# PhilippKath/concentus

Measured on AMD Instinct MI355X. Metric: 48kHz stereo 20ms CELT frames encoded/sec, higher is better.
Workload: dtype int16/int32 fixed-point

## Files before the change

concentus_amd/csrc/celt_enc.h:

```cpp
#pragma once
#include "celt_enc_back.h"

namespace ca {

struct FrameResult { int bytes; u32 final_range; };

template <class L>
CA_DEV void load_state(FrameCtx &fc, L &F, const opusgpu_celt_state *st, int C)
{
    fc.C = C;
    if (st) {
        for (int k = 0; k < 4; k++) fc.hp_mem[k] = st->hp_mem[k];
        fc.rng = st->rng;
        fc.spread_decision = st->spread_decision;
        fc.delayedIntra = st->delayedIntra;
        fc.tonal_average = st->tonal_average;
        fc.lastCodedBands = st->lastCodedBands;
        fc.hf_average = st->hf_average;
        fc.tapset_decision = st->tapset_decision;
        fc.prefilter_period = st->prefilter_period;
        fc.prefilter_gain = st->prefilter_gain;
        fc.prefilter_tapset = st->prefilter_tapset;
        fc.consec_transient = st->consec_transient;
        fc.preemph_memE[0] = st->preemph_memE[0];
// ... 363 lines not shown
    if (!L::IN_IS_GLOBAL)
        for (int c = 0; c < C; c++)
            for (int i = lane(); i < N + OVL; i += LANES) tsig(F, c)[i] = in_ws[c * (N + OVL) + i];
    wave_sync();
  }
  if constexpr (PHASE != 1) {
    int isTransient = 0, shortBlocks = 0, tf_chan = 0, transient_got_disabled = 0;
    i32 tf_estimate = 0;
    if (cfg.complexity >= 1) {
        TransientOut to;
        if constexpr (PHASE == 2) {
            i32 um[2] = {uni(mid->trans_unmask[0]), uni(mid->trans_unmask[1])};
            to = transient_combine(um, C);
        } else {
            to = transient_analysis_wave(F, fc);
        }
        isTransient = to.is_transient;
        tf_estimate = to.tf_estimate;
        tf_chan = to.tf_chan;
    }
    if (ec_tell(enc) + 3 <= total_bits) {
        if (isTransient) shortBlocks = M;
    } else {
        isTransient = 0;
        transient_got_disabled = 1;
    }

    CA_TRACE("transient done isT=%d tf_est=%d", isTransient, tf_estimate); CA_TRACE("");
    CA_STAMP(4);
    const int secondMdct = shortBlocks && cfg.complexity >= 8;
    i32 temporal_vbr = 0;
    for (int mdct_pass = secondMdct ? 0 : 1;;) {
        CA_STAMP(5);
        if constexpr (L::XF_CHANNELS == 1) {
            for (int c = 0; c < C; c++) {
                compute_mdct_channel(F, c, mdct_pass == 0 ? 0 : shortBlocks);
                band_energies_channel(F, c, mdct_pass == 0 ? F.bandLogE2 : F.bandLogE);
                if (mdct_pass != 0) normalise_bands_channel(F, c);
            }
        } else {
            compute_mdcts_wave(F, fc, mdct_pass == 0 ? 0 : shortBlocks);
            CA_STAMP(30);
            band_energies_wave(F, fc, mdct_pass == 0 ? F.bandLogE2 : F.bandLogE);
        }
        CA_STAMP(31);
        if (mdct_pass == 0) {
            for (int k = lane(); k < C * NB; k += LANES) F.bandLogE2[k] = (i16)(F.bandLogE2[k] + (shl16(LM, 10) >> 1));
            wave_sync();
            mdct_pass = 1;
            continue;
        }
        if (mdct_pass == 2) {
            for (int k = lane(); k < C * NB; k += LANES) F.bandLogE2[k] = (i16)(F.bandLogE2[k] + (shl16(LM, 10) >> 1));
            wave_sync();
            tf_estimate = 3277;
            break;
        }
        if constexpr (L::XF_CHANNELS != 1) CA_TAP("freq", F.xf, sizeof(F.xf));
        CA_TAP("bandE", F.bandE, sizeof(F.bandE)); CA_TAP("bandLogE", F.bandLogE, sizeof(F.bandLogE));
        {
            i32 follow = -10240;
            i32 frame_avg = 0;
            i32 offset = shortBlocks ? (shl16(LM, 10) >> 1) : 0;
            for (int i = 0; i < end; i++) {
                follow = (i16)imax(follow - 1024, F.bandLogE[i] - offset);
                if (C == 2) follow = (i16)imax(follow, F.bandLogE[i + NB] - offset);
                frame_avg += follow;
            }
            frame_avg /= end;
            temporal_vbr = (i16)sub16(frame_avg, fc.spec_avg);
            temporal_vbr = imin(3072, imax(-1536, temporal_vbr));
            fc.spec_avg = (i16)(fc.spec_avg + mul16_16_q15(655, temporal_vbr));
        }
        if (!secondMdct) {
            for (int k = lane(); k < C * NB; k += LANES) F.bandLogE2[k] = F.bandLogE[k];
            wave_sync();
        }
        if (!(ec_tell(enc) + 3 <= total_bits && !isTransient && cfg.complexity >= 5)) break;
        i16 *spread_old = F.follower;
        if (lane() == 0) {
            if (C == 1) {
                spread_old[0] = F.oldBandE[0];
                for (int i = 1; i < end; i++) spread_old[i] = (i16)imax(spread_old[i - 1] - 1024, F.oldBandE[i]);
            } else {
                spread_old[0] = (i16)imax(F.oldBandE[0], F.oldBandE[NB]);
                for (int i = 1; i < end; i++)
                    spread_old[i] = (i16)imax(spread_old[i - 1] - 1024, imax(F.oldBandE[i], F.oldBandE[i + NB]));
            }
            for (int i = end - 2; i >= 0; i--) spread_old[i] = (i16)imax(spread_old[i], spread_old[i + 1] - 1024);
        }
        wave_sync();
        i32 mean_diff = 0;
        for (int c = 0; c < C; c++)
            for (int i = 2; i < end - 1; i++) {
                i32 x1 = imax(0, F.bandLogE[i + c * NB]), x2 = imax(0, spread_old[i]);
                mean_diff = add32(mean_diff, imax(0, sub16(x1, x2)));
            }
        mean_diff = mean_diff / (C * (end - 1 - 2));
        wave_sync();
        if (!(mean_diff > 1024)) break;
        isTransient = 1;
        shortBlocks = M;
        mdct_pass = 2;
    }
    if (ec_tell(enc) + 3 <= total_bits) ec_enc_bit_logp(enc, isTransient, 3);

    CA_STAMP(5);
    if constexpr (L::XF_CHANNELS != 1) normalise_bands_wave(F, fc);

    if constexpr (!L::IN_IS_GLOBAL) CA_TAP("X", F.in, 2 * FRAME * 2);
    CA_STAMP(6);
    {
        const i16 *X = frame_X(F);
        if (X != mid->X)
            for (int k = lane(); k < 2 * FRAME; k += LANES) mid->X[k] = X[k];
        MidScalars m;
        m.max_data_bytes = max_data_bytes; m.nbCompressedBytes = nbCompressedBytes; m.nbAvailableBytes = nbAvailableBytes;
        m.effectiveBytes = effectiveBytes; m.vbr_rate = vbr_rate; m.equiv_rate = equiv_rate; m.total_bits = total_bits;
        m.silence = silence; m.pitch_index = pitch_index; m.pf_on = pf_on; m.prefilter_tapset = prefilter_tapset; m.gain1 = gain1;
        m.isTransient = isTransient; m.shortBlocks = shortBlocks; m.tf_chan = tf_chan;
        m.transient_got_disabled = transient_got_disabled; m.tf_estimate = tf_estimate; m.temporal_vbr = temporal_vbr;
        mid_store(F, mid, enc, fc, m);
    }
  }
}

template <class L>
CA_DEVFN void celt_encode_front(L &F, const opusgpu_celt_config &cfg, const opusgpu_celt_state *st_in,
                                opusgpu_celt_state *st_out, const i16 *pcm, FrameMid *mid, StageClock *stage_clock = nullptr)
{
    celt_encode_front_phase<0>(F, cfg, st_in, st_out, pcm, mid, stage_clock, nullptr);
}

template <class L>
CA_DEVFN FrameResult celt_encode_back(L &F, const opusgpu_celt_config &cfg, const FrameMid *mid, opusgpu_celt_state *st_out,
                                      u8 *out, StageClock *stage_clock = nullptr)
{
    (void)stage_clock;
    if (lane() == 0) F.diag = (void *)stage_clock;
    const int C = 2, LM = LM3, end = NB;
    const int celt_vbr = cfg.vbr, constrained_vbr = cfg.constrained_vbr;
// ... 321 lines not shown
```

concentus_amd/csrc/celt_enc_front.h:

```cpp
#pragma once
#include <stddef.h>
#include "celt_math.h"
#include "celt_state.h"
#include "device_tables.h"
#include "mdct_dev.h"
#include "rangecoder.h"

namespace ca {

#if defined(CA_HOST_EMU)
#define CA_DEVFN static inline
#else
#define CA_DEVFN __device__ __forceinline__
#endif

enum { NB = 21, OVL = 120, FRAME = 960, MAXP = 1024, MINP = 15, LM3 = 3, M8 = 8 };
enum { SPREAD_NONE = 0, SPREAD_LIGHT = 1, SPREAD_NORMAL = 2, SPREAD_AGGRESSIVE = 3 };

template <class P, class V> CA_DEV void st0(P p, V v) { if (lane() == 0) *p = v; }

struct __attribute__((aligned(16))) FrontLds {
    enum { IN_IS_GLOBAL = 0, XF_CHANNELS = 2 };
    i32 in[2][FRAME + OVL];
    i32 xf[2][FRAME];
    union {
        i16 raw_pcm[2 * FRAME];
        struct { i16 buf[992]; i16 xlp4[240]; i16 ylp4[484]; i32 xcorr[520]; } pitch;
        i16 trans[2][FRAME + OVL];
        int2 f2[480];
    } s;
    u8 packet[64];
    i32 bandE[2 * NB];
    i16 bandLogE[2 * NB], bandLogE2[2 * NB];
    i16 oldBandE[2 * NB], oldLogE[2 * NB], oldLogE2[2 * NB];
    i16 follower[2 * NB];
    i16 normg[2 * NB];
    i8 normshift[2 * NB];
    i32 scal[16];
    void *diag;
};

#if defined(CA_LANE_FRAME)
enum { LS_SLOTS = 264, LS_PULSES = 240 };
struct FrameMid;
struct BackLds {
    x16_t *x16;
    u8 *packet;
    CA_AS_LDS i16 *col;
    FrameMid *mid;
    void *diag;
    u32 tf_bits;
    int tf_sel;
    u32 ps0[4], ps1[4], ps2[4];
};
#else
struct __attribute__((aligned(16))) BackLds {
    i16 x16[2 * FRAME];
    union {
        struct { i16 tmp[176]; i16 tmp1[176]; } tf;
        struct { i16 y[176]; i32 iy[176]; i16 xabs[176]; } pvq;
    } s;
    u8 packet[1280];
    i32 bandE[2 * NB];
    i16 bandLogE[2 * NB], bandLogE2[2 * NB], error[2 * NB];
    i16 oldBandE[2 * NB], oldLogE[2 * NB], oldLogE2[2 * NB];
    i16 oldE_intra[2 * NB], error_intra[2 * NB];
    i16 follower[2 * NB], noise_floor[NB];
    u8 coarse_save[256];
    i32 offsets[NB], cap[NB], pulses[NB], fine_quant[NB], fine_priority[NB], tf_res[NB];
    i32 bits1[NB], bits2[NB], thresh[NB], trim_offset[NB];
    i32 metric[NB], path0[NB], path1[NB];
    i32 scal[16];
    void *diag;
    i32 pstack[4][8];
};
#endif

struct __attribute__((aligned(16))) Front1Lds {
    enum { IN_IS_GLOBAL = 1, XF_CHANNELS = 2 };
    i32 *in_g;
    i32 xf[2][FRAME];
    union {
        struct { i16 buf[992]; i16 xlp4[240]; i16 ylp4[484]; i32 xcorr[520]; } pitch;
    } s;
    u8 packet[64];
    i32 bandE[2 * NB];
    i16 bandLogE[2 * NB], bandLogE2[2 * NB];
    i16 oldBandE[2 * NB], oldLogE[2 * NB], oldLogE2[2 * NB];
    i32 scal[16];
    void *diag;
};

struct __attribute__((aligned(16))) Front2Lds {
    enum { IN_IS_GLOBAL = 1, XF_CHANNELS = 1 };
    i32 *in_g;
    i16 *x_g;
    i32 xf[1][FRAME];
    union {
        int2 f2[480];
    } s;
    u8 packet[64];
    i32 bandE[2 * NB];
    i16 bandLogE[2 * NB], bandLogE2[2 * NB];
    i16 oldBandE[2 * NB], oldLogE[2 * NB], oldLogE2[2 * NB];
    i16 follower[2 * NB];
    i16 normg[2 * NB];
    i8 normshift[2 * NB];
    i32 scal[16];
    void *diag;
};

CA_DEV i32 *tsig(FrontLds &F, int c) { return F.in[c]; }
CA_DEV i32 *tsig(Front1Lds &F, int c) { return F.in_g + c * (FRAME + OVL); }
CA_DEV i32 *tsig(Front2Lds &F, int c) { return F.in_g + c * (FRAME + OVL); }

CA_DEV i16 *frame_X(FrontLds &F) { return reinterpret_cast<i16 *>(&F.in[0][0]); }
CA_DEV i16 *frame_X(Front2Lds &F) { return F.x_g; }
CA_DEV i16 *frame_pcmf(Front1Lds &F) { return reinterpret_cast<i16 *>(&F.xf[0][0]); }
CA_DEV x16_t *frame_X(BackLds &F) { return F.x16; }
CA_DEV i16 *frame_pcmf(FrontLds &F) { return reinterpret_cast<i16 *>(&F.xf[0][0]); }

struct FrameCtx {
    int C;
    i32 hp_mem[4];
    u32 rng;
    int spread_decision, tonal_average, lastCodedBands, hf_average, tapset_decision;
    i32 delayedIntra;
    int prefilter_period, prefilter_gain, prefilter_tapset, consec_transient;
    i32 preemph_memE[2];
    i32 vbr_reservoir, vbr_drift, vbr_offset, vbr_count, overlap_max;
    int stereo_saving, intensity, spec_avg;
    int stereo_narrow;
    const i32 *hist;
// ... 670 lines not shown
            mean = add32(mean, x2);
            tmp[i] = (i16)(mem0 + pshr32(x2 - mem0, 4));
            mem0 = tmp[i];
        }
        mem0 = 0;
        i32 maxE = 0;
        for (int i = len2 - 1; i >= 0; i--) {
            tmp[i] = (i16)(mem0 + pshr32(tmp[i] - mem0, 3));
            mem0 = tmp[i];
            maxE = imax(maxE, mem0);
        }
        mean = mul16_16(celt_sqrt(mean), celt_sqrt(mul16_16(maxE, len2 >> 1)));
        i32 norm = shl32(len2, 6 + 14) / add32(1, mean >> 1);
        F.scal[4 + c] = norm;
    }
    wave_sync();
    i32 um[2] = {0, 0};
    for (int c = 0; c < C; c++) {
        const i16 *tmp = F.s.trans[c];
        i32 norm = F.scal[4 + c];
        i32 p = 0;
        for (int k = lane(); 12 + 4 * k < len2 - 5; k += LANES) {
            int i = 12 + 4 * k;
            i32 id = imax(0, imin(127, mul16_32_q15((i16)(tmp[i] + 1), norm)));
            p += CLT_inv_table[id];
        }
        i32 unmask = wave_add(p);
        um[c] = 64 * unmask * 4 / (6 * (len2 - 17));
    }
    wave_sync();
    return transient_combine(um, C);
}

template <class L> CA_DEV i32 *xf_row(L &F, int c) { return F.xf[L::XF_CHANNELS == 1 ? 0 : c]; }

template <class L>
CA_DEVFN void compute_mdct_channel(L &F, int c, int shortBlocks)
{
    if (shortBlocks) {
        const MdctTab T = mdct_global_tab<3>();
        mdct_forward_wave<3, 8>(tsig(F, c), F.s.f2, xf_row(F, c), 1, T, lane());
    } else {
        const MdctTab T = mdct_global_tab<0>();
        mdct_forward_wave<0, 1>(tsig(F, c), F.s.f2, xf_row(F, c), 1, T, lane());
    }
}

template <class L>
CA_DEVFN void compute_mdcts_wave(L &F, const FrameCtx &fc, int shortBlocks)
{
    for (int c = 0; c < fc.C; c++) compute_mdct_channel(F, c, shortBlocks);
}

template <class L>
CA_DEVFN void band_energies_channel(L &F, int c, i16 *bandLogE)
{
    const i32 *X = xf_row(F, c);
    i32 *red = reinterpret_cast<i32 *>(F.s.f2);
    constexpr int NCH = 100;
    for (int ch = lane(); ch < NCH; ch += LANES) {
        i32 mx = 0, mn = 0;
#pragma unroll
        for (int u = 0; u < 8; u++) { const i32 v = X[8 * ch + u]; mx = imax(mx, v); mn = imin(mn, v); }
        red[ch] = mx;
        red[NCH + ch] = mn;
    }
    wave_sync();
// ... 34 lines not shown

template <class L>
CA_DEVFN void band_energies_wave(L &F, const FrameCtx &fc, i16 *bandLogE)
{
    for (int c = 0; c < fc.C; c++) band_energies_channel(F, c, bandLogE);
}

template <class L>
CA_DEVFN void normalise_bands_channel(L &F, int c)
{
    i16 *X = frame_X(F);
    const i32 *xf = xf_row(F, c);
    for (int k = c * NB + lane(); k < (c + 1) * NB; k += LANES) {
        i32 bE = F.bandE[k];
        int shift = celt_zlog2(bE) - 13;
        i32 E = (i16)vshr32(bE, shift);
        F.normg[k] = (i16)celt_rcp(shl32(E, 3));
        F.normshift[k] = (i8)shift;
    }
    wave_sync();
    for (int j = lane(); j < (CLT_eband5ms[NB] << LM3); j += LANES) {
        int b = CLT_bin2band[j >> 3] + c * NB;
        X[c * FRAME + j] = (i16)mul16_16_q15(vshr32(xf[j], F.normshift[b] - 1), F.normg[b]);
    }
    wave_sync();
}

template <class L>
CA_DEVFN void normalise_bands_wave(L &F, const FrameCtx &fc)
{
    for (int c = 0; c < fc.C; c++) normalise_bands_channel(F, c);
}

}
```

concentus_amd/csrc/celt_enc_kernel.hip:

```cpp
#include "celt_enc.h"
#include "opusgpu_internal.h"

namespace ca {

__global__ __launch_bounds__(64, 3) void celt_front1_kernel(opusgpu_celt_config cfg, opusgpu_celt_state *states,
                                                            FrameMid *__restrict__ mid, i32 *__restrict__ in_ws, int nframes)
{
    __shared__ Front1Lds F;
    for (int n = blockIdx.x; n < nframes; n += gridDim.x) {
        opusgpu_celt_state *st = states ? states + n : nullptr;
        i32 *in = in_ws + (size_t)n * 2 * (FRAME + OVL);
        if (lane() == 0) F.in_g = in;
        wave_sync();
        celt_encode_front_phase<1>(F, cfg, st, st, nullptr, mid + n, nullptr, in);
        wave_sync();
    }
}

__global__ __launch_bounds__(64, 4) void celt_front2_kernel(opusgpu_celt_config cfg, FrameMid *__restrict__ mid,
                                                            i32 *__restrict__ in_ws, int nframes)
{
    __shared__ Front2Lds F;
    for (int n = blockIdx.x; n < nframes; n += gridDim.x) {
        i32 *in = in_ws + (size_t)n * 2 * (FRAME + OVL);
        if (lane() == 0) { F.in_g = in; F.x_g = mid[n].X; }
        wave_sync();
        celt_encode_front_phase<2>(F, cfg, nullptr, nullptr, nullptr, mid + n, nullptr, in);
        wave_sync();
    }
}

__global__ void celt_state_init_kernel(opusgpu_celt_state *states, int n)
{
    int i = blockIdx.x;
    if (i >= n) return;
    u32 *w = reinterpret_cast<u32 *>(&states[i]);
    for (int k = threadIdx.x; k < (int)(sizeof(opusgpu_celt_state) / 4); k += blockDim.x) w[k] = 0;
    __syncthreads();
    if (threadIdx.x == 0) {
        states[i].spread_decision = SPREAD_NORMAL;
        states[i].delayedIntra = 1;
        states[i].tonal_average = 256;
    }
    for (int k = threadIdx.x; k < 2 * NB; k += blockDim.x) {
        states[i].oldLogE[k] = -28672;
        states[i].oldLogE2[k] = -28672;
    }
}

}

// ... 106 lines not shown
```

concentus_amd/csrc/mdct_dev.h:

```cpp
#pragma once
#include "fixmath.h"
#include "device_tables.h"

namespace ca {

struct MdctTab {
    const u32 *tw;
    const u32 *trig;
    const i16 *bitrev;
    const i16 *window;
    const i16 *bitrev_sw;
};

template <int SHIFT>
CA_DEV MdctTab mdct_global_tab()
{
    MdctTab t;
    t.tw = CLT_fft_tw_packed;
    t.trig = SHIFT == 0 ? CLT_mdct_trig_packed0 : SHIFT == 1 ? CLT_mdct_trig_packed1
           : SHIFT == 2 ? CLT_mdct_trig_packed2 : CLT_mdct_trig_packed3;
    t.bitrev = SHIFT == 0 ? CLT_fft_bitrev480 : SHIFT == 1 ? CLT_fft_bitrev240
             : SHIFT == 2 ? CLT_fft_bitrev120 : CLT_fft_bitrev60;
    t.window = CLT_window120;
    t.bitrev_sw = CLT_fft_bitrev480_sw;
// ... 17 lines not shown
    for (int i = tid; i < 120; i += nthreads) L.window[i] = g.window[i];
    MdctTab t;
    t.tw = L.tw; t.trig = L.trig; t.bitrev = L.bitrev; t.window = L.window;
    t.bitrev_sw = g.bitrev_sw;
    return t;
}

struct cpx { i32 r, i; };
CA_DEV cpx ld(const int2 *p) { int2 v = *p; return cpx{v.x, v.y}; }
CA_DEV void st(int2 *p, cpx v) { *p = make_int2(v.r, v.i); }
CA_DEV i32 lo16(u32 p) { return (i32)(i16)(p & 0xffff); }
CA_DEV i32 hi16(u32 p) { return (i32)p >> 16; }
#define CA_SMUL(x, t) mul16_32_q15((t), (x))

CA_DEV cpx c_mul(cpx a, u32 tw)
{
    i32 tr = lo16(tw), ti = hi16(tw);
    cpx m;
    m.r = sub32(CA_SMUL(a.r, tr), CA_SMUL(a.i, ti));
    m.i = add32(CA_SMUL(a.r, ti), CA_SMUL(a.i, tr));
    return m;
}
CA_DEV cpx c_add(cpx a, cpx b) { return cpx{add32(a.r, b.r), add32(a.i, b.i)}; }
CA_DEV cpx c_sub(cpx a, cpx b) { return cpx{sub32(a.r, b.r), sub32(a.i, b.i)}; }

#if defined(CA_HOST_EMU)
#define CA_FFT_ROLLED
CA_DEV int fft_lane(int lane) { return lane; }
#else
#define CA_FFT_ROLLED _Pragma("clang loop unroll(disable)")
CA_DEV int fft_lane(int lane) { asm volatile("" : "+v"(lane)); return lane; }
#endif

template <int SHIFT>
CA_DEV int fsw(int e)
{
    if constexpr (SHIFT == 0) {
        constexpr unsigned long long LUT = CLT_FSW_LUT;
        const int s = (int)(LUT >> ((e >> 3) & 60)) & 30;
        return e ^ s ^ ((e >> 2) & 4);
    } else {
        return e;
    }
}

template <int SW, int P, int M>
CA_DEV void fft_members(int e, int (&a)[P])
{
    if constexpr (SW != 0) {
#pragma unroll
        for (int c = 0; c < P; c++) a[c] = e + c * M;
    } else if constexpr (M == 8) {
        const int A = e ^ ((int)(CLT_FSW_LUT >> ((e >> 3) & 60)) & 30);
#pragma unroll
        for (int c = 0; c < P; c++) a[c] = A ^ ((8 * c) ^ (4 * (c >> 1)));
    } else {
        static_assert(M % 32 == 0, "members whole blocks apart");
        const unsigned long long W = CLT_FSW_LUT >> ((e >> 3) & 60);
        const int E = e ^ ((e >> 2) & 4);
#pragma unroll
        for (int c = 0; c < P; c++) a[c] = (E + c * M) ^ ((int)(W >> (4 * ((c * M) >> 5))) & 30);
    }
}

struct cpx2 { cpx a, b; };
CA_DEV cpx2 ld2(const int2 *p)
{
    const int4 v = *reinterpret_cast<const int4 *>(p);
    return cpx2{cpx{v.x, v.y}, cpx{v.z, v.w}};
}
CA_DEV void st2(int2 *p, cpx a, cpx b)
{
    int4 v;
    v.x = a.r; v.y = a.i; v.z = b.r; v.w = b.i;
    *reinterpret_cast<int4 *>(p) = v;
}

template <int NFFT, int B>
CA_DEV void fft_radix4_first(int2 *x, int lane)
{
    constexpr int CNT = B * NFFT / 4;
    for (int idx = lane; idx < CNT; idx += LANES) {
        int2 *f = x + 4 * idx;
        cpx x0 = ld(f), x1 = ld(f + 1), x2 = ld(f + 2), x3 = ld(f + 3);
        cpx s0 = c_sub(x0, x2);
        x0 = c_add(x0, x2);
        cpx s1 = c_add(x1, x3);
        x2 = c_sub(x0, s1);
        x0 = c_add(x0, s1);
        s1 = c_sub(x1, x3);
        st(f, x0);
        st(f + 2, x2);
        st(f + 1, cpx{add32(s0.r, s1.i), sub32(s0.i, s1.r)});
        st(f + 3, cpx{sub32(s0.r, s1.i), add32(s0.i, s1.r)});
    }
}

template <int NFFT, int B>
CA_DEV void fft_radix2_m4(int2 *x, int lane)
{
    constexpr int CNT = B * NFFT / 2;
    constexpr i32 TW = 23170;
    for (int idx = lane; idx < CNT; idx += LANES) {
        int g = idx >> 2, k = idx & 3;
        int2 *f = x + 8 * g + k;
        cpx a = ld(f), b = ld(f + 4), t;
        if (k == 0) {
            t = b;
        } else if (k == 1) {
            t.r = CA_SMUL(add32(b.r, b.i), TW);
            t.i = CA_SMUL(sub32(b.i, b.r), TW);
        } else if (k == 2) {
            t.r = b.i;
            t.i = neg32(b.r);
        } else {
            t.r = CA_SMUL(sub32(b.i, b.r), TW);
            t.i = CA_SMUL(sub32(neg32(b.i), b.r), TW);
        }
        st(f + 4, c_sub(a, t));
        st(f, c_add(a, t));
    }
}

template <int SHIFT>
CA_DEV void fft_first8(int2 *x, int lane)
{
    constexpr int NFFT = 480 >> SHIFT;
    constexpr i32 TW = 23170;
    lane = fft_lane(lane);
    for (int g = lane; g < NFFT / 8; g += LANES) {
        cpx v[8];
        const int A = fsw<SHIFT>(8 * g);
#pragma unroll
        for (int q = 0; q < 4; q++) {
            const cpx2 t = ld2(x + (A ^ (2 * q)));
            v[2 * q] = t.a;
            v[2 * q + 1] = t.b;
        }
#pragma unroll
        for (int h = 0; h < 2; h++) {
            cpx x0 = v[4 * h], x1 = v[4 * h + 1], x2 = v[4 * h + 2], x3 = v[4 * h + 3];
            cpx s0 = c_sub(x0, x2);
            x0 = c_add(x0, x2);
            cpx s1 = c_add(x1, x3);
            x2 = c_sub(x0, s1);
            x0 = c_add(x0, s1);
            s1 = c_sub(x1, x3);
            v[4 * h] = x0;
            v[4 * h + 2] = x2;
            v[4 * h + 1] = cpx{add32(s0.r, s1.i), sub32(s0.i, s1.r)};
            v[4 * h + 3] = cpx{sub32(s0.r, s1.i), add32(s0.i, s1.r)};
        }
        {
            cpx t, b;
            b = v[4]; t = b;
            v[4] = c_sub(v[0], t); v[0] = c_add(v[0], t);
            b = v[5]; t.r = CA_SMUL(add32(b.r, b.i), TW); t.i = CA_SMUL(sub32(b.i, b.r), TW);
            v[5] = c_sub(v[1], t); v[1] = c_add(v[1], t);
            b = v[6]; t.r = b.i; t.i = neg32(b.r);
            v[6] = c_sub(v[2], t); v[2] = c_add(v[2], t);
            b = v[7]; t.r = CA_SMUL(sub32(b.i, b.r), TW); t.i = CA_SMUL(sub32(neg32(b.i), b.r), TW);
            v[7] = c_sub(v[3], t); v[3] = c_add(v[3], t);
        }
#pragma unroll
        for (int q = 0; q < 4; q++) st2(x + (A ^ (2 * q)), v[2 * q], v[2 * q + 1]);
    }
}

template <int NFFT, int B, int M>
CA_DEV void fft_radix4(int2 *x, const u32 *tw, int lane)
{
    constexpr int G = NFFT / (4 * M);
    constexpr int TWS = G * (480 / NFFT);
    constexpr int CNT = B * NFFT / 4;
    constexpr int SW = (NFFT == 480 && B == 1) ? 0 : 1;
    lane = fft_lane(lane);
    CA_FFT_ROLLED
    for (int idx = lane; idx < CNT; idx += LANES) {
        int blk = idx / (G * M), r = idx % (G * M);
        int g = r / M, j = r % M;
        const int e = blk * NFFT + g * 4 * M + j;
        int m[4];
        fft_members<SW, 4, M>(e, m);
        int2 *f0p = x + m[0], *f1p = x + m[1], *f2p = x + m[2], *f3p = x + m[3];
        cpx f0 = ld(f0p);
        cpx a = c_mul(ld(f1p), tw[j * TWS]);
        cpx b = c_mul(ld(f2p), tw[2 * j * TWS]);
        cpx c = c_mul(ld(f3p), tw[3 * j * TWS]);
        cpx d5 = c_sub(f0, b);
        f0 = c_add(f0, b);
        cpx s3 = c_add(a, c);
        cpx s4 = c_sub(a, c);
        st(f2p, c_sub(f0, s3));
        st(f0p, c_add(f0, s3));
        st(f1p, cpx{add32(d5.r, s4.i), sub32(d5.i, s4.r)});
        st(f3p, cpx{sub32(d5.r, s4.i), add32(d5.i, s4.r)});
    }
}

template <int NFFT, int B, int M>
CA_DEV void fft_radix3(int2 *x, const u32 *tw, int lane)
{
    constexpr int G = NFFT / (3 * M);
    constexpr int TWS = G * (480 / NFFT);
    constexpr int CNT = B * NFFT / 3;
    constexpr int SW = (NFFT == 480 && B == 1) ? 0 : 1;
    constexpr i32 EPI3 = -28378;
    lane = fft_lane(lane);
    CA_FFT_ROLLED
    for (int idx = lane; idx < CNT; idx += LANES) {
        int blk = idx / (G * M), r = idx % (G * M);
        int g = r / M, j = r % M;
        const int e = blk * NFFT + g * 3 * M + j;
        int m[3];
        fft_members<SW, 3, M>(e, m);
        int2 *f0p = x + m[0], *f1p = x + m[1], *f2p = x + m[2];
        cpx f0 = ld(f0p);
        cpx a = c_mul(ld(f1p), tw[j * TWS]);
        cpx b = c_mul(ld(f2p), tw[2 * j * TWS]);
        cpx s3 = c_add(a, b);
        cpx s0 = c_sub(a, b);
        cpx f1{sub32(f0.r, s3.r >> 1), sub32(f0.i, s3.i >> 1)};
        s0.r = CA_SMUL(s0.r, EPI3);
        s0.i = CA_SMUL(s0.i, EPI3);
        st(f0p, c_add(f0, s3));
        st(f2p, cpx{add32(f1.r, s0.i), sub32(f1.i, s0.r)});
        st(f1p, cpx{sub32(f1.r, s0.i), add32(f1.i, s0.r)});
    }
}

template <int NFFT, int B, int M>
CA_DEV void fft_radix5(int2 *x, const u32 *tw, int lane)
{
    constexpr int G = NFFT / (5 * M);
    constexpr int TWS = G * (480 / NFFT);
    constexpr int CNT = B * NFFT / 5;
    constexpr int SW = (NFFT == 480 && B == 1) ? 0 : 1;
    constexpr i32 YAR = 10126, YAI = -31164, YBR = -26510, YBI = -19261;
    lane = fft_lane(lane);
    CA_FFT_ROLLED
    for (int idx = lane; idx < CNT; idx += LANES) {
        int blk = idx / (G * M), r = idx % (G * M);
        int g = r / M, u = r % M;
        const int e = blk * NFFT + g * 5 * M + u;
        int m[5];
        fft_members<SW, 5, M>(e, m);
        int2 *f0p = x + m[0], *f1p = x + m[1], *f2p = x + m[2], *f3p = x + m[3], *f4p = x + m[4];
        cpx s0 = ld(f0p);
        cpx s1 = c_mul(ld(f1p), tw[u * TWS]);
        cpx s2 = c_mul(ld(f2p), tw[2 * u * TWS]);
        cpx s3 = c_mul(ld(f3p), tw[3 * u * TWS]);
        cpx s4 = c_mul(ld(f4p), tw[4 * u * TWS]);
        cpx s7 = c_add(s1, s4), s10 = c_sub(s1, s4);
        cpx s8 = c_add(s2, s3), s9 = c_sub(s2, s3);
        st(f0p, cpx{add32(s0.r, add32(s7.r, s8.r)), add32(s0.i, add32(s7.i, s8.i))});
        cpx s5, s6, s11, s12;
        s5.r = add32(add32(s0.r, CA_SMUL(s7.r, YAR)), CA_SMUL(s8.r, YBR));
        s5.i = add32(add32(s0.i, CA_SMUL(s7.i, YAR)), CA_SMUL(s8.i, YBR));
        s6.r = add32(CA_SMUL(s10.i, YAI), CA_SMUL(s9.i, YBI));
        s6.i = sub32(neg32(CA_SMUL(s10.r, YAI)), CA_SMUL(s9.r, YBI));
        st(f1p, c_sub(s5, s6));
        st(f4p, c_add(s5, s6));
        s11.r = add32(add32(s0.r, CA_SMUL(s7.r, YBR)), CA_SMUL(s8.r, YAR));
        s11.i = add32(add32(s0.i, CA_SMUL(s7.i, YBR)), CA_SMUL(s8.i, YAR));
        s12.r = add32(neg32(CA_SMUL(s10.i, YBI)), CA_SMUL(s9.i, YAI));
        s12.i = sub32(CA_SMUL(s10.r, YBI), CA_SMUL(s9.r, YAI));
        st(f2p, c_add(s11, s12));
        st(f3p, c_sub(s11, s12));
    }
}

template <int SHIFT, int B> CA_DEV int fft_at(int e) { return fsw<(SHIFT == 0 && B == 1) ? 0 : 1>(e); }
template <int SHIFT, int B> CA_DEV void fft_put(int2 *x, int e, cpx v) { st(x + fft_at<SHIFT, B>(e), v); }
template <int SHIFT, int B> CA_DEV cpx fft_get(const int2 *x, int e) { return ld(x + fft_at<SHIFT, B>(e)); }

template <int SHIFT, int B>
CA_DEV void fft_wave(int2 *x, const u32 *tw, int lane)
{
    constexpr int NFFT = 480 >> SHIFT;
    if constexpr (SHIFT == 0 && B == 1) {
        fft_first8<0>(x, lane);                 wave_sync();
        fft_radix4<NFFT, B, 8>(x, tw, lane);    wave_sync();
        fft_radix3<NFFT, B, 32>(x, tw, lane);   wave_sync();
        fft_radix5<NFFT, B, 96>(x, tw, lane);   wave_sync();
        return;
    }
    fft_radix4_first<NFFT, B>(x, lane);
    wave_sync();
    if constexpr (SHIFT == 0) {
        fft_radix2_m4<NFFT, B>(x, lane);        wave_sync();
        fft_radix4<NFFT, B, 8>(x, tw, lane);    wave_sync();
        fft_radix3<NFFT, B, 32>(x, tw, lane);   wave_sync();
        fft_radix5<NFFT, B, 96>(x, tw, lane);   wave_sync();
    } else if constexpr (SHIFT == 1) {
        fft_radix4<NFFT, B, 4>(x, tw, lane);    wave_sync();
        fft_radix3<NFFT, B, 16>(x, tw, lane);   wave_sync();
        fft_radix5<NFFT, B, 48>(x, tw, lane);   wave_sync();
    } else if constexpr (SHIFT == 2) {
        fft_radix2_m4<NFFT, B>(x, lane);        wave_sync();
        fft_radix3<NFFT, B, 8>(x, tw, lane);    wave_sync();
        fft_radix5<NFFT, B, 24>(x, tw, lane);   wave_sync();
    } else {
        fft_radix3<NFFT, B, 4>(x, tw, lane);    wave_sync();
        fft_radix5<NFFT, B, 12>(x, tw, lane);   wave_sync();
    }
}

template <int SHIFT>
CA_DEV cpx mdct_fwd_pre(const i32 *in, int i, const MdctTab &T)
{
    constexpr int N2 = 960 >> SHIFT, N4 = N2 / 2;
    constexpr int OV = 120, OV2 = 60, Q = 30;
    constexpr int SCALE_SHIFT = (8 - SHIFT) - 1;
    const int a = OV2 + 2 * i, b = N2 - 1 + OV2 - 2 * i;
    i32 re, im;
    if (i < Q) {
        i32 w1 = T.window[OV2 + 2 * i], w2 = T.window[OV2 - 1 - 2 * i];
        re = add32(mul16_32_q15(w2, in[a + N2]), mul16_32_q15(w1, in[b]));
        im = sub32(mul16_32_q15(w1, in[a]), mul16_32_q15(w2, in[b - N2]));
    } else if (i < N4 - Q) {
        re = in[b];
        im = in[a];
    } else {
        int k = i - (N4 - Q);
        i32 w1 = T.window[2 * k], w2 = T.window[OV - 1 - 2 * k];
        re = add32(neg32(mul16_32_q15(w1, in[a - N2])), mul16_32_q15(w2, in[b]));
        im = add32(mul16_32_q15(w2, in[a]), mul16_32_q15(w1, in[b + N2]));
    }
    u32 t = T.trig[i];
    i32 t0 = lo16(t), t1 = hi16(t);
    i32 yr = sub32(CA_SMUL(re, t0), CA_SMUL(im, t1));
    i32 yi = add32(CA_SMUL(im, t0), CA_SMUL(re, t1));
    return cpx{pshr32(mul16_32_q16(17476, yr), SCALE_SHIFT), pshr32(mul16_32_q16(17476, yi), SCALE_SHIFT)};
}

enum { FFT_PAIRS = 240, FFT_PAIR_STEP = LANES >= 60 ? 60 : LANES };
CA_DEV int fft_pair_input(int n) { return n < 120 ? n : n + 120; }
// ... 1 lines not shown
template <int SHIFT, int B>
CA_DEV void mdct_forward_wave(const i32 *sin, int2 *f2, i32 *dst, int dstride, const MdctTab &T, int lane)
{
    const u32 *trig = T.trig;
    const i16 *bitrev = T.bitrev;
    constexpr int N2 = 960 >> SHIFT, N4 = N2 / 2, NFFT = N4;
    if constexpr (SHIFT == 0 && B == 1) {
        static_assert(FFT_PAIRS % FFT_PAIR_STEP == 0, "whole trips");
        if (lane < FFT_PAIR_STEP) {
            CA_FFT_ROLLED
            for (int n0 = 0; n0 < FFT_PAIRS; n0 += FFT_PAIR_STEP) {
                const int i = fft_pair_input(n0 + lane);
                const cpx a = mdct_fwd_pre<SHIFT>(sin, i, T), b = mdct_fwd_pre<SHIFT>(sin, i + 120, T);
                st2(f2 + T.bitrev_sw[i], a, b);
            }
        }
    } else {
        for (int idx = lane; idx < B * N4; idx += LANES) {
            int blk = idx / N4, i = idx % N4;
            fft_put<SHIFT, B>(f2, blk * NFFT + bitrev[i], mdct_fwd_pre<SHIFT>(sin + blk * N2, i, T));
        }
    }
    wave_sync();
    fft_wave<SHIFT, B>(f2, T.tw, lane);
    for (int idx = lane; idx < B * N4; idx += LANES) {
        int blk = idx / N4, i = idx % N4;
        cpx f = fft_get<SHIFT, B>(f2, blk * NFFT + i);
        u32 t = trig[i];
        i32 t0 = lo16(t), t1 = hi16(t);
        dst[((2 * i) * B + blk) * dstride] = sub32(CA_SMUL(f.i, t1), CA_SMUL(f.r, t0));
        dst[((N2 - 1 - 2 * i) * B + blk) * dstride] = add32(CA_SMUL(f.r, t1), CA_SMUL(f.i, t0));
    }
    wave_sync();
}

template <int SHIFT, int B>
CA_DEV void mdct_backward_wave(const i32 *src, int sstride, int2 *f2, i32 *out, const MdctTab &T, int lane)
{
    const u32 *trig = T.trig;
    const i16 *bitrev = T.bitrev;
    constexpr int N2 = 960 >> SHIFT, N4 = N2 / 2, NFFT = N4;
    constexpr int OV = 120, OV2 = 60;
    auto pre = [&](int blk, int i) {
        i32 x1 = src[((2 * i) * B + blk) * sstride];
        i32 x2 = src[((N2 - 1 - 2 * i) * B + blk) * sstride];
        u32 t = trig[i];
        i32 t0 = lo16(t), t1 = hi16(t);
        i32 yr = add32(CA_SMUL(x2, t0), CA_SMUL(x1, t1));
        i32 yi = sub32(CA_SMUL(x1, t0), CA_SMUL(x2, t1));
        return cpx{yi, yr};
    };
    if constexpr (SHIFT == 0 && B == 1) {
        if (lane < FFT_PAIR_STEP) {
            CA_FFT_ROLLED
            for (int n0 = 0; n0 < FFT_PAIRS; n0 += FFT_PAIR_STEP) {
                const int i = fft_pair_input(n0 + lane);
                st2(f2 + T.bitrev_sw[i], pre(0, i), pre(0, i + 120));
            }
        }
    } else {
        for (int idx = lane; idx < B * N4; idx += LANES) {
            int blk = idx / N4, i = idx % N4;
            fft_put<SHIFT, B>(f2, blk * NFFT + bitrev[i], pre(blk, i));
        }
    }
    wave_sync();
// ... 25 lines not shown
```

Before: 9.644 million.

## Process both channels jointly in front2 MDCT, band energy and normalisation

Replaces the per-channel MDCT/band-energy/normalise loop in the single-xf front2 layout with joint two-channel versions. The FFT stages take a channel-count parameter so each stage handles both channels in one wave pass, halving the number of barrier-separated stages. The MDCT output is rotated in place into the FFT buffer, which is unioned with xf. Band energies use a two-level reduction over 8-bin chunks instead of per-band serial loops. This adds LDS use (a reduction buffer and shift array, guarded by a static_assert for 16 waves per CU) and more register pressure from the staged post-rotation.

```diff
diff --git a/concentus_amd/csrc/celt_enc.h b/concentus_amd/csrc/celt_enc.h
--- a/concentus_amd/csrc/celt_enc.h
+++ b/concentus_amd/csrc/celt_enc.h
@@ -419,12 +419,12 @@
     i32 temporal_vbr = 0;
     for (int mdct_pass = secondMdct ? 0 : 1;;) {
         CA_STAMP(5);
-        if constexpr (L::XF_CHANNELS == 1) {
-            for (int c = 0; c < C; c++) {
-                compute_mdct_channel(F, c, mdct_pass == 0 ? 0 : shortBlocks);
-                band_energies_channel(F, c, mdct_pass == 0 ? F.bandLogE2 : F.bandLogE);
-                if (mdct_pass != 0) normalise_bands_channel(F, c);
-            }
+        if (mdct_pass == 2) CA_COUNT("front_mdct_redo", 1);
+        else if (mdct_pass == 1 && shortBlocks) CA_COUNT("front_mdct_short", 1);
+        if constexpr (L::JOINT_CHANNELS) {
+            compute_mdcts_joint(F, mdct_pass == 0 ? 0 : shortBlocks);
+            band_energies_joint(F, mdct_pass == 0 ? F.bandLogE2 : F.bandLogE);
+            if (mdct_pass != 0) normalise_bands_joint(F);
         } else {
             compute_mdcts_wave(F, fc, mdct_pass == 0 ? 0 : shortBlocks);
             CA_STAMP(30);
@@ -443,7 +443,7 @@
             tf_estimate = 3277;
             break;
         }
-        if constexpr (L::XF_CHANNELS != 1) CA_TAP("freq", F.xf, sizeof(F.xf));
+        if constexpr (!L::JOINT_CHANNELS) CA_TAP("freq", F.xf, sizeof(F.xf));
         CA_TAP("bandE", F.bandE, sizeof(F.bandE)); CA_TAP("bandLogE", F.bandLogE, sizeof(F.bandLogE));
         {
             i32 follow = -10240;
@@ -493,7 +493,7 @@
     if (ec_tell(enc) + 3 <= total_bits) ec_enc_bit_logp(enc, isTransient, 3);
 
     CA_STAMP(5);
-    if constexpr (L::XF_CHANNELS != 1) normalise_bands_wave(F, fc);
+    if constexpr (!L::JOINT_CHANNELS) normalise_bands_wave(F, fc);
 
     if constexpr (!L::IN_IS_GLOBAL) CA_TAP("X", F.in, 2 * FRAME * 2);
     CA_STAMP(6);
diff --git a/concentus_amd/csrc/celt_enc_front.h b/concentus_amd/csrc/celt_enc_front.h
--- a/concentus_amd/csrc/celt_enc_front.h
+++ b/concentus_amd/csrc/celt_enc_front.h
@@ -20,7 +20,7 @@
 template <class P, class V> CA_DEV void st0(P p, V v) { if (lane() == 0) *p = v; }
 
 struct __attribute__((aligned(16))) FrontLds {
-    enum { IN_IS_GLOBAL = 0, XF_CHANNELS = 2 };
+    enum { IN_IS_GLOBAL = 0, JOINT_CHANNELS = 0 };
     i32 in[2][FRAME + OVL];
     i32 xf[2][FRAME];
     union {
@@ -77,7 +77,7 @@
 #endif
 
 struct __attribute__((aligned(16))) Front1Lds {
-    enum { IN_IS_GLOBAL = 1, XF_CHANNELS = 2 };
+    enum { IN_IS_GLOBAL = 1, JOINT_CHANNELS = 0 };
     i32 *in_g;
     i32 xf[2][FRAME];
     union {
@@ -92,13 +92,15 @@
 };
 
 struct __attribute__((aligned(16))) Front2Lds {
-    enum { IN_IS_GLOBAL = 1, XF_CHANNELS = 1 };
+    enum { IN_IS_GLOBAL = 1, JOINT_CHANNELS = 1 };
     i32 *in_g;
     i16 *x_g;
-    i32 xf[1][FRAME];
     union {
-        int2 f2[480];
+        int2 f2[2][FFT_CH_STRIDE];
+        i32 xf[2][FRAME];
     } s;
+    i32 red[200];
+    i16 eshift[2 * NB];
     u8 packet[64];
     i32 bandE[2 * NB];
     i16 bandLogE[2 * NB], bandLogE2[2 * NB];
@@ -835,7 +837,7 @@
     return transient_combine(um, C);
 }
 
-template <class L> CA_DEV i32 *xf_row(L &F, int c) { return F.xf[L::XF_CHANNELS == 1 ? 0 : c]; }
+template <class L> CA_DEV i32 *xf_row(L &F, int c) { return F.xf[c]; }
 
 template <class L>
 CA_DEVFN void compute_mdct_channel(L &F, int c, int shortBlocks)
@@ -936,4 +938,97 @@
     for (int c = 0; c < fc.C; c++) normalise_bands_channel(F, c);
 }
 
-}
+template <class L>
+CA_DEVFN void compute_mdcts_joint(L &F, int shortBlocks)
+{
+    if (shortBlocks) {
+        const MdctTab T = mdct_global_tab<3>();
+        mdct_forward_wave2<3, 8>(tsig(F, 0), FRAME + OVL, F.s.f2[0], T, lane());
+    } else {
+        const MdctTab T = mdct_global_tab<0>();
+        mdct_forward_wave2<0, 1>(tsig(F, 0), FRAME + OVL, F.s.f2[0], T, lane());
+    }
+}
+
+template <class L>
+CA_DEVFN void band_energies_joint(L &F, i16 *bandLogE)
+{
+    const i32 *X = F.s.xf[0];
+    i32 *red = F.red;
+    constexpr int NCH = 100;
+    for (int q = lane(); q < 2 * NCH; q += LANES) {
+        const int c = q >= NCH ? 1 : 0;
+        const i32 *x = X + c * (FRAME - 8 * NCH) + 8 * q;
+        i32 mx = 0, mn = 0;
+#pragma unroll
+        for (int u = 0; u < 8; u++) { const i32 v = x[u]; mx = imax(mx, v); mn = imin(mn, v); }
+        const u32 neg = 0u - (u32)mn;
+        red[q] = (i32)((u32)mx > neg ? (u32)mx : neg);
+    }
+    wave_sync();
+    for (int k = lane(); k < 2 * NB; k += LANES) {
+        const int c = k >= NB ? 1 : 0, b = k - c * NB;
+        u32 mag = 0;
+        for (int ch = CLT_eband5ms[b]; ch < CLT_eband5ms[b + 1]; ch++) { const u32 m = (u32)red[c * NCH + ch]; mag = m > mag ? m : mag; }
+        i32 maxval = (i32)mag;
+        if (mag == 0x80000000u) {
+            maxval = 0;
+            for (int j = CLT_eband5ms[b] << LM3; j < (CLT_eband5ms[b + 1] << LM3); j++) maxval = imax(maxval, X[c * FRAME + j]);
+        }
+        F.eshift[k] = (i16)(maxval > 0 ? celt_ilog2(maxval) - 14 + (((CLT_logN400[b] >> 3) + LM3 + 1) >> 1) : 0x7fff);
+    }
+    wave_sync();
+    for (int q = lane(); q < 2 * NCH; q += LANES) {
+        const int c = q >= NCH ? 1 : 0;
+        const i32 *x = X + c * (FRAME - 8 * NCH) + 8 * q;
+        const int shift = F.eshift[CLT_bin2band[q - c * NCH] + c * NB];
+        i32 sum = 0;
+        if (shift != 0x7fff) {
+#pragma unroll
+            for (int u = 0; u < 8; u++) {
+                const i32 xv = x[u];
+                const i32 v = shift > 0 ? (i16)(xv >> shift) : (i16)shl32(xv, -shift);
+                sum = mac16_16(sum, v, v);
+            }
+        }
+        red[q] = sum;
+    }
+    wave_sync();
+    for (int k = lane(); k < 2 * NB; k += LANES) {
+        const int c = k >= NB ? 1 : 0, b = k - c * NB;
+        const int shift = F.eshift[k];
+        i32 E = 1;
+        if (shift != 0x7fff) {
+            i32 sum = 0;
+            for (int ch = CLT_eband5ms[b]; ch < CLT_eband5ms[b + 1]; ch++) sum = add32(sum, red[c * NCH + ch]);
+            E = add32(1, vshr32(celt_sqrt(sum), -shift));
+        }
+        F.bandE[k] = E;
+        bandLogE[k] = (i16)(celt_log2(shl32(E, 2)) - shl16(CLT_eMeans[b], 6));
+    }
+    wave_sync();
+}
+
+template <class L>
+CA_DEVFN void normalise_bands_joint(L &F)
+{
+    i16 *X = frame_X(F);
+    const i32 *xf = F.s.xf[0];
+    constexpr int NBIN = 800;
+    for (int k = lane(); k < 2 * NB; k += LANES) {
+        i32 bE = F.bandE[k];
+        int shift = celt_zlog2(bE) - 13;
+        i32 E = (i16)vshr32(bE, shift);
+        F.normg[k] = (i16)celt_rcp(shl32(E, 3));
+        F.normshift[k] = (i8)shift;
+    }
+    wave_sync();
+    for (int q = lane(); q < 2 * NBIN; q += LANES) {
+        const int c = q >= NBIN ? 1 : 0, j = q - c * NBIN;
+        int b = CLT_bin2band[j >> 3] + c * NB;
+        X[c * FRAME + j] = (i16)mul16_16_q15(vshr32(xf[c * FRAME + j], F.normshift[b] - 1), F.normg[b]);
+    }
+    wave_sync();
+}
+
+}
diff --git a/concentus_amd/csrc/celt_enc_kernel.hip b/concentus_amd/csrc/celt_enc_kernel.hip
--- a/concentus_amd/csrc/celt_enc_kernel.hip
+++ b/concentus_amd/csrc/celt_enc_kernel.hip
@@ -17,6 +17,7 @@
     }
 }
 
+static_assert(sizeof(Front2Lds) * 16 <= 160 * 1024, "celt_front2_kernel: 16 wavefronts per CU");
 __global__ __launch_bounds__(64, 4) void celt_front2_kernel(opusgpu_celt_config cfg, FrameMid *__restrict__ mid,
                                                             i32 *__restrict__ in_ws, int nframes)
 {
diff --git a/concentus_amd/csrc/mdct_dev.h b/concentus_amd/csrc/mdct_dev.h
--- a/concentus_amd/csrc/mdct_dev.h
+++ b/concentus_amd/csrc/mdct_dev.h
@@ -73,6 +73,20 @@
 CA_DEV int fft_lane(int lane) { asm volatile("" : "+v"(lane)); return lane; }
 #endif
 
+enum { FFT_CH_STRIDE = 480 };
+template <int NCH, int CNT>
+CA_DEV int fft_split(int &idx)
+{
+    static_assert(NCH == 1 || NCH == 2, "one transform or a pair");
+    if constexpr (NCH == 1) {
+        return 0;
+    } else {
+        const int ch = idx >= CNT ? 1 : 0;
+        idx -= ch * CNT;
+        return ch * FFT_CH_STRIDE;
+    }
+}
+
 template <int SHIFT>
 CA_DEV int fsw(int e)
 {
@@ -117,12 +131,13 @@
     *reinterpret_cast<int4 *>(p) = v;
 }
 
-template <int NFFT, int B>
+template <int NFFT, int B, int NCH = 1>
 CA_DEV void fft_radix4_first(int2 *x, int lane)
 {
     constexpr int CNT = B * NFFT / 4;
-    for (int idx = lane; idx < CNT; idx += LANES) {
-        int2 *f = x + 4 * idx;
+    for (int idx0 = lane; idx0 < NCH * CNT; idx0 += LANES) {
+        int idx = idx0;
+        int2 *f = x + fft_split<NCH, CNT>(idx) + 4 * idx;
         cpx x0 = ld(f), x1 = ld(f + 1), x2 = ld(f + 2), x3 = ld(f + 3);
         cpx s0 = c_sub(x0, x2);
         x0 = c_add(x0, x2);
@@ -137,14 +152,16 @@
     }
 }
 
-template <int NFFT, int B>
+template <int NFFT, int B, int NCH = 1>
 CA_DEV void fft_radix2_m4(int2 *x, int lane)
 {
     constexpr int CNT = B * NFFT / 2;
     constexpr i32 TW = 23170;
-    for (int idx = lane; idx < CNT; idx += LANES) {
+    for (int idx0 = lane; idx0 < NCH * CNT; idx0 += LANES) {
+        int idx = idx0;
+        int2 *xc = x + fft_split<NCH, CNT>(idx);
         int g = idx >> 2, k = idx & 3;
-        int2 *f = x + 8 * g + k;
+        int2 *f = xc + 8 * g + k;
         cpx a = ld(f), b = ld(f + 4), t;
         if (k == 0) {
             t = b;
@@ -163,13 +180,15 @@
     }
 }
 
-template <int SHIFT>
-CA_DEV void fft_first8(int2 *x, int lane)
+template <int SHIFT, int NCH = 1>
+CA_DEV void fft_first8(int2 *xb, int lane)
 {
     constexpr int NFFT = 480 >> SHIFT;
     constexpr i32 TW = 23170;
     lane = fft_lane(lane);
-    for (int g = lane; g < NFFT / 8; g += LANES) {
+    for (int g0 = lane; g0 < NCH * (NFFT / 8); g0 += LANES) {
+        int g = g0;
+        int2 *x = xb + fft_split<NCH, NFFT / 8>(g);
         cpx v[8];
         const int A = fsw<SHIFT>(8 * g);
 #pragma unroll
@@ -208,8 +227,8 @@
     }
 }
 
-template <int NFFT, int B, int M>
-CA_DEV void fft_radix4(int2 *x, const u32 *tw, int lane)
+template <int NFFT, int B, int M, int NCH = 1>
+CA_DEV void fft_radix4(int2 *xb, const u32 *tw, int lane)
 {
     constexpr int G = NFFT / (4 * M);
     constexpr int TWS = G * (480 / NFFT);
@@ -217,7 +236,9 @@
     constexpr int SW = (NFFT == 480 && B == 1) ? 0 : 1;
     lane = fft_lane(lane);
     CA_FFT_ROLLED
-    for (int idx = lane; idx < CNT; idx += LANES) {
+    for (int idx0 = lane; idx0 < NCH * CNT; idx0 += LANES) {
+        int idx = idx0;
+        int2 *x = xb + fft_split<NCH, CNT>(idx);
         int blk = idx / (G * M), r = idx % (G * M);
         int g = r / M, j = r % M;
         const int e = blk * NFFT + g * 4 * M + j;
@@ -239,8 +260,8 @@
     }
 }
 
-template <int NFFT, int B, int M>
-CA_DEV void fft_radix3(int2 *x, const u32 *tw, int lane)
+template <int NFFT, int B, int M, int NCH = 1>
+CA_DEV void fft_radix3(int2 *xb, const u32 *tw, int lane)
 {
     constexpr int G = NFFT / (3 * M);
     constexpr int TWS = G * (480 / NFFT);
@@ -249,7 +270,9 @@
     constexpr i32 EPI3 = -28378;
     lane = fft_lane(lane);
     CA_FFT_ROLLED
-    for (int idx = lane; idx < CNT; idx += LANES) {
+    for (int idx0 = lane; idx0 < NCH * CNT; idx0 += LANES) {
+        int idx = idx0;
+        int2 *x = xb + fft_split<NCH, CNT>(idx);
         int blk = idx / (G * M), r = idx % (G * M);
         int g = r / M, j = r % M;
         const int e = blk * NFFT + g * 3 * M + j;
@@ -270,8 +293,8 @@
     }
 }
 
-template <int NFFT, int B, int M>
-CA_DEV void fft_radix5(int2 *x, const u32 *tw, int lane)
+template <int NFFT, int B, int M, int NCH = 1>
+CA_DEV void fft_radix5(int2 *xb, const u32 *tw, int lane)
 {
     constexpr int G = NFFT / (5 * M);
     constexpr int TWS = G * (480 / NFFT);
@@ -280,7 +303,9 @@
     constexpr i32 YAR = 10126, YAI = -31164, YBR = -26510, YBI = -19261;
     lane = fft_lane(lane);
     CA_FFT_ROLLED
-    for (int idx = lane; idx < CNT; idx += LANES) {
+    for (int idx0 = lane; idx0 < NCH * CNT; idx0 += LANES) {
+        int idx = idx0;
+        int2 *x = xb + fft_split<NCH, CNT>(idx);
         int blk = idx / (G * M), r = idx % (G * M);
         int g = r / M, u = r % M;
         const int e = blk * NFFT + g * 5 * M + u;
@@ -315,35 +340,35 @@
 template <int SHIFT, int B> CA_DEV void fft_put(int2 *x, int e, cpx v) { st(x + fft_at<SHIFT, B>(e), v); }
 template <int SHIFT, int B> CA_DEV cpx fft_get(const int2 *x, int e) { return ld(x + fft_at<SHIFT, B>(e)); }
 
-template <int SHIFT, int B>
+template <int SHIFT, int B, int NCH = 1>
 CA_DEV void fft_wave(int2 *x, const u32 *tw, int lane)
 {
     constexpr int NFFT = 480 >> SHIFT;
     if constexpr (SHIFT == 0 && B == 1) {
-        fft_first8<0>(x, lane);                 wave_sync();
-        fft_radix4<NFFT, B, 8>(x, tw, lane);    wave_sync();
-        fft_radix3<NFFT, B, 32>(x, tw, lane);   wave_sync();
-        fft_radix5<NFFT, B, 96>(x, tw, lane);   wave_sync();
+        fft_first8<0, NCH>(x, lane);                 wave_sync();
+        fft_radix4<NFFT, B, 8, NCH>(x, tw, lane);    wave_sync();
+        fft_radix3<NFFT, B, 32, NCH>(x, tw, lane);   wave_sync();
+        fft_radix5<NFFT, B, 96, NCH>(x, tw, lane);   wave_sync();
         return;
     }
-    fft_radix4_first<NFFT, B>(x, lane);
+    fft_radix4_first<NFFT, B, NCH>(x, lane);
     wave_sync();
     if constexpr (SHIFT == 0) {
-        fft_radix2_m4<NFFT, B>(x, lane);        wave_sync();
-        fft_radix4<NFFT, B, 8>(x, tw, lane);    wave_sync();
-        fft_radix3<NFFT, B, 32>(x, tw, lane);   wave_sync();
-        fft_radix5<NFFT, B, 96>(x, tw, lane);   wave_sync();
+        fft_radix2_m4<NFFT, B, NCH>(x, lane);        wave_sync();
+        fft_radix4<NFFT, B, 8, NCH>(x, tw, lane);    wave_sync();
+        fft_radix3<NFFT, B, 32, NCH>(x, tw, lane);   wave_sync();
+        fft_radix5<NFFT, B, 96, NCH>(x, tw, lane);   wave_sync();
     } else if constexpr (SHIFT == 1) {
-        fft_radix4<NFFT, B, 4>(x, tw, lane);    wave_sync();
-        fft_radix3<NFFT, B, 16>(x, tw, lane);   wave_sync();
-        fft_radix5<NFFT, B, 48>(x, tw, lane);   wave_sync();
+        fft_radix4<NFFT, B, 4, NCH>(x, tw, lane);    wave_sync();
+        fft_radix3<NFFT, B, 16, NCH>(x, tw, lane);   wave_sync();
+        fft_radix5<NFFT, B, 48, NCH>(x, tw, lane);   wave_sync();
     } else if constexpr (SHIFT == 2) {
-        fft_radix2_m4<NFFT, B>(x, lane);        wave_sync();
-        fft_radix3<NFFT, B, 8>(x, tw, lane);    wave_sync();
-        fft_radix5<NFFT, B, 24>(x, tw, lane);   wave_sync();
-    } else {
-        fft_radix3<NFFT, B, 4>(x, tw, lane);    wave_sync();
-        fft_radix5<NFFT, B, 12>(x, tw, lane);   wave_sync();
+        fft_radix2_m4<NFFT, B, NCH>(x, lane);        wave_sync();
+        fft_radix3<NFFT, B, 8, NCH>(x, tw, lane);    wave_sync();
+        fft_radix5<NFFT, B, 24, NCH>(x, tw, lane);   wave_sync();
+    } else {
+        fft_radix3<NFFT, B, 4, NCH>(x, tw, lane);    wave_sync();
+        fft_radix5<NFFT, B, 12, NCH>(x, tw, lane);   wave_sync();
     }
 }
 
@@ -411,6 +436,98 @@
         dst[((N2 - 1 - 2 * i) * B + blk) * dstride] = add32(CA_SMUL(f.r, t1), CA_SMUL(f.i, t0));
     }
     wave_sync();
+}
+
+#if defined(CA_HOST_EMU)
+#define CA_POST_UNROLL
+#else
+#define CA_POST_UNROLL _Pragma("unroll")
+#endif
+template <int SHIFT, int B>
+CA_DEV void mdct_forward_wave2(const i32 *sin, int sin_stride, int2 *f2, const MdctTab &T, int lane)
+{
+    const u32 *trig = T.trig;
+    const i16 *bitrev = T.bitrev;
+    constexpr int NCH = 2;
+    constexpr int N2 = 960 >> SHIFT, N4 = N2 / 2, NFFT = N4;
+    static_assert(B * N4 == FFT_CH_STRIDE, "a whole frame per channel");
+    if constexpr (SHIFT == 0 && B == 1) {
+        if (lane < FFT_PAIR_STEP) {
+            CA_FFT_ROLLED
+            for (int n0 = 0; n0 < NCH * FFT_PAIRS; n0 += FFT_PAIR_STEP) {
+                const int ch = n0 >= FFT_PAIRS ? 1 : 0;
+                const i32 *in = sin + ch * sin_stride;
+                const int i = fft_pair_input(n0 - ch * FFT_PAIRS + lane);
+                const cpx a = mdct_fwd_pre<SHIFT>(in, i, T), b = mdct_fwd_pre<SHIFT>(in, i + 120, T);
+                st2(f2 + ch * FFT_CH_STRIDE + T.bitrev_sw[i], a, b);
+            }
+        }
+    } else {
+        for (int idx0 = lane; idx0 < NCH * B * N4; idx0 += LANES) {
+            int idx = idx0;
+            const int off = fft_split<NCH, B * N4>(idx);
+            const i32 *in = sin + (off / FFT_CH_STRIDE) * sin_stride;
+            int blk = idx / N4, i = idx % N4;
+            fft_put<SHIFT, B>(f2 + off, blk * NFFT + bitrev[i], mdct_fwd_pre<SHIFT>(in + blk * N2, i, T));
+        }
+    }
+    wave_sync();
+    fft_wave<SHIFT, B, NCH>(f2, T.tw, lane);
+    auto rotate = [&](const int2 *x, int e, int i, i32 &ya, i32 &yb) {
+        cpx f = fft_get<SHIFT, B>(x, e);
+        u32 tt = trig[i];
+        i32 t0 = lo16(tt), t1 = hi16(tt);
+        ya = sub32(CA_SMUL(f.i, t1), CA_SMUL(f.r, t0));
+        yb = add32(CA_SMUL(f.r, t1), CA_SMUL(f.i, t0));
+    };
+    if constexpr (SHIFT == 0 && B == 1) {
+        constexpr int SET = 64, PER = SET / LANES, NBLK = NFFT / 32, MID = NBLK / 2;
+        static_assert(SET % LANES == 0 && NBLK == 2 * MID + 1, "block pairs g, 14 - g around a middle block");
+        CA_FFT_ROLLED
+        for (int t = 0; t < NCH * MID + 1; t++) {
+            const int last = t == NCH * MID, tc = t >= MID ? 1 : 0, g = last ? MID : t - tc * MID;
+            i32 ya[PER], yb[PER];
+            CA_POST_UNROLL
+            for (int u = 0; u < PER; u++) {
+                const int m = lane + u * LANES, hi = m >> 5;
+                const int ch = last ? hi : tc, i = 32 * (hi && !last ? NBLK - 1 - g : g) + (m & 31);
+                rotate(f2 + ch * FFT_CH_STRIDE, i, i, ya[u], yb[u]);
+            }
+            wave_sync();
+            CA_POST_UNROLL
+            for (int u = 0; u < PER; u++) {
+                const int m = lane + u * LANES, hi = m >> 5;
+                const int ch = last ? hi : tc, i = 32 * (hi && !last ? NBLK - 1 - g : g) + (m & 31);
+                i32 *dst = reinterpret_cast<i32 *>(f2 + ch * FFT_CH_STRIDE);
+                dst[2 * i] = ya[u];
+                dst[N2 - 1 - 2 * i] = yb[u];
+            }
+            wave_sync();
+        }
+    } else {
+        constexpr int PER = (B * N4 + LANES - 1) / LANES;
+        CA_FFT_ROLLED
+        for (int ch = 0; ch < NCH; ch++) {
+            int2 *x = f2 + ch * FFT_CH_STRIDE;
+            i32 ya[PER], yb[PER];
+            CA_POST_UNROLL
+            for (int u = 0; u < PER; u++) {
+                const int idx = lane + u * LANES;
+                if (idx < B * N4) rotate(x, idx, idx % N4, ya[u], yb[u]);
+            }
+            wave_sync();
+            CA_POST_UNROLL
+            for (int u = 0; u < PER; u++) {
+                const int idx = lane + u * LANES, blk = idx / N4, i = idx % N4;
+                if (idx < B * N4) {
+                    i32 *dst = reinterpret_cast<i32 *>(x);
+                    dst[(2 * i) * B + blk] = ya[u];
+                    dst[(N2 - 1 - 2 * i) * B + blk] = yb[u];
+                }
+            }
+            wave_sync();
+        }
+    }
 }
 
 template <int SHIFT, int B>
```

New measurement: 9.925 million, median of 6. 1.03x the previous value.
